# sizhe-li/neural-jacobian-field

Hardware: AMD Instinct MI355X
Metric: rendered rays/s (64 samples/ray, 256^2 image) (higher is better)
Workload: dtype f32 (v_mfma_f32_32x32x2_f32: exact fp32 products, fp32 accumulate -- the reference's arithmetic)

## Files before the change

### include/njf_hip.h

```cpp
#ifndef NJF_HIP_H
#define NJF_HIP_H

#include <stddef.h>
#include <stdint.h>

#ifdef __cplusplus
extern "C" {
#endif

#define NJF_ABI_VERSION 20
#define NJF_MAX_ACTION_DIM 10
#define NJF_HIDDEN 128
#define NJF_LATENT 512
#define NJF_PE_DIM 63
#define NJF_ZDIM 384

#define NJF_RESNET_CHUNKS 22
#define NJF_RESNET_CHUNKS_F16 12
#define NJF_CHUNK_FLOATS 8192
#define NJF_RESNET_W_FLOATS (NJF_RESNET_CHUNKS * NJF_CHUNK_FLOATS)
#define NJF_RESNET_B_FLOATS (10 * 128 + 32)
#define NJF_COLOR_W_FLOATS NJF_CHUNK_FLOATS
#define NJF_COLOR_B_FLOATS (64 + 32)
#define NJF_TRANSFORMER_CHUNKS 7
#define NJF_TRANSFORMER_W_FLOATS (NJF_TRANSFORMER_CHUNKS * NJF_CHUNK_FLOATS)
#define NJF_TRANSFORMER_B_FLOATS (3 * 256 + 32)
#define NJF_QDIM 64

#define NJF_PRECISION_F32 0
#define NJF_PRECISION_F16X2 1
#define NJF_PRECISION_F16F6 2

#define NJF_PRECISION_F16 3

#define NJF_PRECISION_MIXED(d, j) ((d) | (((j) + 1) << 4))

#define NJF_JACOBIAN_NONE 0
#define NJF_JACOBIAN_MLP 1
#define NJF_JACOBIAN_TRANSFORMER 2

typedef struct NjfResnetFcWeights {
  const float* lin_in_w;
  const float* lin_in_b;
  const float* fc0_w[5];
  const float* fc0_b[5];
  const float* fc1_w[5];
  const float* fc1_b[5];
  const float* lin_z_w[3];
  const float* lin_z_b[3];
  const float* lin_out_w;
  const float* lin_out_b;
  int d_out;
} NjfResnetFcWeights;

typedef struct NjfColorHeadWeights {
  const float* w0; const float* b0;
// ... 395 lines not shown
```

### neural-jacobian-field_amd/csrc/njf_device.h

```cpp
#pragma once
#include <hip/hip_runtime.h>
#include <stdint.h>

__device__ __forceinline__ float relu_bits(float x) { return __int_as_float(max(__float_as_int(x), 0)); }

typedef float f32x16 __attribute__((ext_vector_type(16)));
typedef float f32x4 __attribute__((ext_vector_type(4)));
typedef _Float16 f16x8 __attribute__((ext_vector_type(8)));
typedef _Float16 f16x16 __attribute__((ext_vector_type(16)));
typedef _Float16 f16x32 __attribute__((ext_vector_type(32)));
typedef int i32x8 __attribute__((ext_vector_type(8)));
typedef int i32x4 __attribute__((ext_vector_type(4)));
typedef int i32x2 __attribute__((ext_vector_type(2)));
typedef unsigned u32x6 __attribute__((ext_vector_type(6)));

#define PREC_F32 0
#define PREC_F16X2 1
#define PREC_F16F6 2
#define PREC_F16 3

#define NJF_WAVES 4
#define NJF_THREADS (NJF_WAVES * 64)
#define NJF_CHUNK 8192

#define NJF_STREAM_BUFFERS 2
#define LDS_CTR_FLOATS 0
#define LDS_W0 0
#define LDS_W1 NJF_CHUNK
#define LDS_BIAS (NJF_STREAM_BUFFERS * NJF_CHUNK)
#define LDS_BIAS_FLOATS 2752
#define LDS_BIAS_FLOATS_PROPOSAL 1344
#define LDS_SCRATCH_PER_WAVE 528
#define LDS_FLOATS_RENDER (LDS_BIAS + LDS_BIAS_FLOATS + LDS_CTR_FLOATS)
#define LDS_FLOATS_PROPOSAL (LDS_BIAS + LDS_BIAS_FLOATS_PROPOSAL + NJF_WAVES * LDS_SCRATCH_PER_WAVE + LDS_CTR_FLOATS)
#define LDS_SCRATCH_PROPOSAL (LDS_BIAS + LDS_BIAS_FLOATS_PROPOSAL)

extern __shared__ __attribute__((aligned(16))) float njf_lds[];

__device__ __forceinline__ float mfma_step(float a, float b, f32x16& c) {
  c = __builtin_amdgcn_mfma_f32_32x32x2f32(a, b, c, 0, 0, 0);
  return 0.f;
}

#ifdef NJF_STAMPS
#define NJF_STAMP_SLOTS 1024
#ifdef NJF_STAMPS_PROPOSAL
#define NJF_STAMP_BASE LDS_FLOATS_PROPOSAL
#define NJF_STAMP_LOGS_PROPOSAL true
#else
#define NJF_STAMP_BASE LDS_FLOATS_RENDER
#define NJF_STAMP_LOGS_PROPOSAL false
#endif
__device__ unsigned njf_stamp_out[NJF_STAMP_SLOTS];
#define NJF_STAMP_FIELD int stamp_i;
#define NJF_STAMP_INIT(st) (st).stamp_i = -1
#define NJF_STAMP(st, tag)                                                                                   \
  do {                                                                                                       \
    if ((st).stamp_i >= 0 && (st).stamp_i < NJF_STAMP_SLOTS) {                                               \
      njf_lds[NJF_STAMP_BASE + (st).stamp_i] =                                                               \
          __uint_as_float(((unsigned)(tag) << 24) | ((unsigned)__builtin_readcyclecounter() & 0xffffffu));   \
      (st).stamp_i += 1;                                                                                     \
    }                                                                                                        \
  } while (0)
#define NJF_STAMP_P(st, tag) do { if (NJF_STAMP_LOGS_PROPOSAL) NJF_STAMP(st, tag); } while (0)
// ... 129 lines not shown
}
template <bool RELU>
__device__ __forceinline__ void split_pair_u(float x0, float x1, unsigned& hu, unsigned& lu) {
  if (RELU) {
    x0 = relu_bits(x0);
    x1 = relu_bits(x1);
  }
  const f16x2 hp = {(_Float16)x0, (_Float16)x1};
  hu = __builtin_bit_cast(unsigned, hp);
  asm("v_fma_mixlo_f16 %0, -%1, 1.0, %2 op_sel:[0,0,0] op_sel_hi:[1,0,0]" : "=v"(lu) : "v"(hu), "v"(x0));
  asm("v_fma_mixhi_f16 %0, -%1, 1.0, %2 op_sel:[1,0,0] op_sel_hi:[1,0,0]" : "+v"(lu) : "v"(hu), "v"(x1));
}

typedef short s16x2 __attribute__((ext_vector_type(2)));
template <bool RELU>
__device__ __forceinline__ unsigned pack_pair_f16(float x0, float x1) {
  typedef float f32x2 __attribute__((ext_vector_type(2)));
  const f32x2 xp = {x0, x1};
  const f16x2 hp = __builtin_convertvector(xp, f16x2);
  if constexpr (RELU) {
    const s16x2 z = {0, 0};
    return __builtin_bit_cast(unsigned, __builtin_elementwise_max(__builtin_bit_cast(s16x2, hp), z));
  } else {
    return __builtin_bit_cast(unsigned, hp);
  }
}

#define F6_HI 0
#define F6_P1 16384
#define F6_P2 24576
#define F6_SCALE 28672


template <int PREC, int MBO, int NKB, int KB0, bool RELU, int KBI, class ST>
__device__ __forceinline__ void mma_chunk(ST& st, const float* __restrict__ wl, int lane,
                                          const f32x16 (&in)[KBI], f32x16 (&out)[MBO]) {
  constexpr bool SPREAD = MBO == 4 && (NKB == 2 || (PREC == PREC_F16 && NKB == 4)) && NJF_DMA_ROUNDS == 8;
  if constexpr (!SPREAD) stream_flush(st);
  if constexpr (PREC == PREC_F32) {
    const float* base = wl + lane * 4;
#pragma unroll
    for (int kb = 0; kb < NKB; ++kb) {
#pragma unroll
      for (int q = 0; q < 4; ++q) {
        f32x4 a[MBO];
#pragma unroll
        for (int m = 0; m < MBO; ++m) a[m] = *(const f32x4*)(base + ((kb * 4 + q) * MBO + m) * 256);
        if constexpr (SPREAD) {
          if (kb * 4 + q < 4) {
            dma_issue(st, 2 * (kb * 4 + q));
            dma_issue(st, 2 * (kb * 4 + q) + 1);
          }
        }
#pragma unroll
        for (int e = 0; e < 4; ++e) {
          float b = in[KB0 + kb][q * 4 + e];
          if (RELU) b = relu_bits(b);
#pragma unroll
          for (int m = 0; m < MBO; ++m) out[m] = __builtin_amdgcn_mfma_f32_32x32x2f32(a[m][e], b, out[m], 0, 0, 0);
        }
      }
    }
  } else if constexpr (PREC == PREC_F16F6 && MBO == 4 && NKB == 2) {
    typedef __attribute__((address_space(3))) const char* lds_ptr;
    const lds_ptr wb = (lds_ptr)(const char*)wl;
    lds_ptr p16 = wb + lane * 16;
    lds_ptr p8 = wb + lane * 8;
    asm volatile("" : "+v"(p16), "+v"(p8));
    unsigned bh[4][4], bl[4][4], mx[4];
#pragma unroll
    for (int p = 0; p < 4; ++p) {
// ... 690 lines not shown
    for (int m = 0; m < 4; ++m)
#pragma unroll
      for (int q = 0; q < 2; ++q) {
        u32x4 o;
#pragma unroll
        for (int e = 0; e < 4; ++e) o[e] = pack_pair_f16<DO_RELU>(v[m][8 * q + 2 * e], v[m][8 * q + 2 * e + 1]);
        *(u32x4*)(d16 + 16 * m + 8 * q) = o;
      }
  } else {
#pragma unroll
  for (int m = 0; m < 4; ++m)
#pragma unroll
    for (int q = 0; q < 4; ++q) {
      f32x4 o;
#pragma unroll
      for (int e = 0; e < 4; ++e) o[e] = DO_RELU ? fmaxf(v[m][4 * q + e], 0.f) : v[m][4 * q + e];
      *(f32x4*)(dst + 16 * m + 4 * q) = o;
    }
  }
  if (mask != nullptr) {
    unsigned w[2] = {0u, 0u};
#pragma unroll
    for (int m = 0; m < 4; ++m)
#pragma unroll
      for (int r = 0; r < 16; ++r) {
        const unsigned b = (unsigned)min(max(__float_as_int(v[m][r]), 0), 1);
        w[m >> 1] |= b << (16 * (m & 1) + r);
      }
    typedef unsigned u32x2 __attribute__((ext_vector_type(2)));
    *(u32x2*)mask = u32x2{w[0], w[1]};
  }
}

template <int PREC, bool DUMP = false, int SHARED = 0, class ST>
__device__ __forceinline__ void resnet_tile(ST& st, const float* __restrict__ bias,
                                            const float* __restrict__ gz, const PointGeom& g,
                                            const f32x16 (&pe)[2], int wave, int lane, f32x16 (&out)[1],
                                            ActDump dump = ActDump{nullptr, nullptr, 0}, const TileShareF16* share = nullptr) {
  static_assert(SHARED == 0 || (PREC == PREC_F16 && !DUMP), "the shared tile state exists for the plain-fp16 inference kernels");
  const int hh = lane >> 5;
  constexpr bool FUSED = PREC == PREC_F32 && !DUMP;
  f32x16 h[4], net[4];
#pragma unroll
  for (int m = 0; m < 4; ++m) h[m] = (f32x16)(0.f);
  if (DUMP && dump.pe != nullptr) {
#pragma unroll
    for (int kb = 0; kb < 2; ++kb)
#pragma unroll
      for (int q = 0; q < 4; ++q) {
        f32x4 o;
#pragma unroll
        for (int e = 0; e < 4; ++e) o[e] = pe[kb][4 * q + e];
        *(f32x4*)(dump.pe + 16 * kb + 4 * q) = o;
      }
  }
  {
    const float* wl = stream_step(st, wave, lane);
    if constexpr ((SHARED & 1) != 0) mma_lin_in_f16_packed(st, wl, lane, share->pe, h);
    else if constexpr (FUSED) mma_chunk_gather_f32<0, false, 2>(st, wl, lane, pe, h, gz, g);
    else mma_chunk<PREC, 4, 2, 0, false, 2>(st, wl, lane, pe, h);
  }
  if constexpr (PREC == PREC_F16) {
    static_assert(!DUMP, "the plain-fp16 mode is an inference mode (training forwards dump fp32-class activations)");
    Footprint fp_net;
    if constexpr ((SHARED & 2) != 0) point_footprint(g, fp_net);
    for (int blk = 0; blk < 5; ++blk) {
      if (blk < 3) {
        NJF_STAMP(st, 4);
        if constexpr ((SHARED & 2) != 0) add_hoisted_latent_f16<4>((const _Float16*)map_at<PREC>(gz, blk * 128), g, hh, h, &fp_net);
        else add_hoisted_latent<4, PREC>(map_at<PREC>(gz, blk * 128), g, lane, h);
        NJF_STAMP(st, 5);
      }
// ... 15 lines not shown
      NJF_STAMP(st, 4);
      add_hoisted_latent<4, PREC>(gz + blk * 128, g, lane, h);
      NJF_STAMP(st, 5);
    }
    if (DUMP) dump_vec128<true>(dump_layer(dump, 2 * blk), h, dump.mask ? dump.mask + (size_t)(2 * blk) * (dump.stride / 32) : nullptr, dump.half);
    const float* bl = bias + blk * 256;
    bias_init<4, true, PREC>(bl, hh, net);
    {
      {
        const float* wl = stream_step(st, wave, lane);
        mma_chunk<PREC, 4, 2, 0, true, 4>(st, wl, lane, h, net);
      }
      {
        const float* wl = stream_step(st, wave, lane);
        mma_chunk<PREC, 4, 2, 2, true, 4>(st, wl, lane, h, net);
      }
    }
    if (DUMP) dump_vec128<true>(dump_layer(dump, 2 * blk + 1), net, dump.mask ? dump.mask + (size_t)(2 * blk + 1) * (dump.stride / 32) : nullptr, dump.half);
    bias_init<4, false, PREC>(bl + 128, hh, h);
    {
      {
        const float* wl = stream_step(st, wave, lane);
        mma_chunk<PREC, 4, 2, 0, true, 4>(st, wl, lane, net, h);
      }
      {
        const float* wl = stream_step(st, wave, lane);
        bool plain = true;
        if constexpr (FUSED) {
          if (blk < 2) {
            mma_chunk_gather_f32<2, true, 4>(st, wl, lane, net, h, gz + (blk + 1) * 128, g);
            plain = false;
          }
        }
        if (plain) mma_chunk<PREC, 4, 2, 2, true, 4>(st, wl, lane, net, h);
      }
    }
    if (DUMP && dump.feat != nullptr) dump_vec128<false>(dump.feat + (size_t)blk * dump.stride, h);
  }
  if (DUMP) dump_vec128<true>(dump_layer(dump, 10), h, dump.mask ? dump.mask + (size_t)10 * (dump.stride / 32) : nullptr, dump.half);
  bias_init<1, true, PREC>(bias + 1280, hh, out);
  {
    const float* wl = stream_step(st, wave, lane);
    mma_chunk<PREC, 1, 4, 0, true, 4>(st, wl, lane, h, out);
  }
}

struct ColorDump {
  float* in;
  float* act;
  size_t stride;
};

template <bool DO_RELU>
__device__ __forceinline__ void dump_vec32(float* __restrict__ dst, const f32x16 (&v)[2]) {
#pragma unroll
  for (int m = 0; m < 2; ++m)
#pragma unroll
    for (int q = 0; q < 4; ++q) {
      f32x4 o;
#pragma unroll
      for (int e = 0; e < 4; ++e) o[e] = DO_RELU ? fmaxf(v[m][4 * q + e], 0.f) : v[m][4 * q + e];
      *(f32x4*)(dst + 16 * m + 4 * q) = o;
    }
}

template <int PREC, bool DUMP = false, class ST>
__device__ __forceinline__ void color_tile(ST& st, const float* __restrict__ bias, const f32x16 (&cin)[1],
                                           int wave, int lane, f32x16 (&rgb)[1],
                                           ColorDump dump = ColorDump{nullptr, nullptr, 0}) {
  const int hh = lane >> 5;
  const float* wl = stream_step(st, wave, lane);
  f32x16 a[2], b[2];
  a[0] = (f32x16)(0.f);
  a[1] = (f32x16)(0.f);
  mma_chunk<PREC, 2, 1, 0, false, 1>(st, wl, lane, cin, a);
  bias_init<2, true, PREC>(bias, hh, b);
  mma_chunk<PREC, 2, 2, 0, true, 2>(st, wl + 2048, lane, a, b);
  bias_init<1, true, PREC>(bias + 64, hh, rgb);
  mma_chunk<PREC, 1, 2, 0, true, 2>(st, wl + 6144, lane, b, rgb);
  if (DUMP && dump.in != nullptr) {
#pragma unroll
    for (int q = 0; q < 4; ++q) {
      f32x4 o;
#pragma unroll
      for (int e = 0; e < 4; ++e) o[e] = cin[0][4 * q + e];
      *(f32x4*)(dump.in + 4 * q) = o;
    }
    dump_vec32<true>(dump.act, a);
    dump_vec32<true>(dump.act + dump.stride, b);
  }
}

__device__ __forceinline__ float erf_branchless(float a) {
  const float t = fabsf(a), s = a * a;
  float r = fmaf(-1.72853470e-5f, t, 3.83197126e-4f);
  const float u = fmaf(-3.88396438e-3f, t, 2.42546219e-2f);
  r = fmaf(r, s, u);
  r = fmaf(r, t, -1.06777877e-1f);
  r = fmaf(r, t, -6.34846687e-1f);
  r = fmaf(r, t, -1.28717512e-1f);
  r = fmaf(r, t, -t);
  const float hi = copysignf(1.0f - __builtin_amdgcn_exp2f(r * 1.4426950408889634f), a);
  float q = -5.96761703e-4f;
  q = fmaf(q, s, 4.99119423e-3f);
  q = fmaf(q, s, -2.67681349e-2f);
  q = fmaf(q, s, 1.12819925e-1f);
  q = fmaf(q, s, -3.76125336e-1f);
  q = fmaf(q, s, 1.28379166e-1f);
  const float lo = fmaf(q, a, a);
  return t > 0.927734375f ? hi : lo;
}

// ... 198 lines not shown
```

### neural-jacobian-field_amd/csrc/njf_kernels.hip

```cpp
#include <hip/hip_runtime.h>
#include <math.h>
#include <stdint.h>

#include <atomic>
#include <type_traits>

#include "../../include/njf_hip.h"
#include "njf_device.h"

enum {
  NJF_OK = 0,
  NJF_E_NULL = -1,
  NJF_E_SHAPE = -2,
  NJF_E_ACTION_DIM = -3,
  NJF_E_SAMPLES = -4,
  NJF_E_DOUT = -5,
  NJF_E_MODE = -6,
  NJF_E_GMAP = -7,
  NJF_E_VALUE = -8,
};

extern "C" int njf_abi_version(void) { return NJF_ABI_VERSION; }
extern "C" int njf_rays_per_workgroup(void) { return NJF_WAVES; }

// ... 188 lines not shown
      const int ip = lane & 31, kh = lane >> 5;
      const int f = 16 * L.mb * ((ip >> 2) & 1) + 16 * m + (ip & 3) + 4 * (ip >> 3);
      const int k = 16 * L.kb * kh + 8 * t + i8;
      const float v = pack_source(L, f, k);
      const _Float16 hi = (_Float16)v;
      const _Float16 lo = (_Float16)(v - (float)hi);
      const size_t o = ((size_t)(t * L.mb + m) * 2) * 512 + lane * 8 + i8;
      dst[o] = hi;
      dst[o + 512] = lo;
    }
  }
  if (L.bdst != nullptr && blockIdx.x == 0) {
    for (int f = threadIdx.x; f < 32 * L.mb; f += blockDim.x) L.bdst[f] = pack_bias_entry(L, f);
  }
}

__global__ void pack_layer_kernel(PackLayer L) { pack_layer_body(L); }

#define NJF_PACK_BATCH 24
struct PackBatch {
  PackLayer l[NJF_PACK_BATCH];
  unsigned char f6[NJF_PACK_BATCH];
  int count;
};

__global__ void pack_batch_kernel(PackBatch B) {
  const int k = blockIdx.y;
  if (B.f6[k]) pack_layer_f16f6_body(B.l[k]);
  else pack_layer_body(B.l[k]);
}

__global__ void fill_kernel(float* p, int n, float v) {
  for (int i = blockIdx.x * blockDim.x + threadIdx.x; i < n; i += gridDim.x * blockDim.x) p[i] = v;
}

__host__ __device__ inline int njf_hoist_layout(int precision) {
  return precision == NJF_PRECISION_F16F6 ? 1 : (precision == NJF_PRECISION_F16 ? 2 : 0);
}
__host__ __device__ inline int njf_hoist_position(int f, int mb_count, int layout) {
  const int hh = f / (16 * mb_count), r = f % (16 * mb_count);
  const int m = r >> 4;
  if (layout == 0) {
    const int q = (r >> 2) & 3, e = r & 3;
    return 32 * m + 8 * q + 4 * hh + e;
  }
  if (layout == 2) {
    const int q = (r >> 3) & 1, e = r & 7;
    return 32 * m + 16 * q + 8 * hh + e;
  }
  const int e = (r >> 2) & 3, i = r & 3;
  return 16 * mb_count * hh + 16 * m + 4 * i + e;
}

extern "C" int njf_hoisted_channel(int feature, int block_channels, int precision) {
  if (block_channels < 32 || (block_channels & 31) || feature < 0 || feature >= block_channels) return NJF_E_SHAPE;
  if (!valid_base_precision(precision)) return NJF_E_MODE;
  return njf_hoist_position(feature, block_channels / 32, njf_hoist_layout(precision));
}

__global__ void pack_linz_kernel(const float* w0, const float* w1, const float* w2, const float* b0, const float* b1,
                                 const float* b2, float* wz, int ld, float* bz, int layout, const float* fold0,
                                 const float* fold1) {
  const int n = 3 * 128 * 512;
  for (int i = blockIdx.x * blockDim.x + threadIdx.x; i < n; i += gridDim.x * blockDim.x) {
    const int c = i % 384, k = i / 384;
    const int l = c >> 7, f = c & 127;
// ... 46 lines not shown
  }
  if (g_pack_scope != nullptr && g_pack_scope->s == s) {
    g_pack_scope->add(L, f6);
    return;
  }
  if (f6) pack_layer_f16f6_kernel<<<64, 256, 0, s>>>(L);
  else pack_layer_kernel<<<(n + 255) / 256, 256, 0, s>>>(L);
}

extern "C" int njf_pack_resnetfc_ld(const NjfResnetFcWeights* src, float* w_out, float* b_out, float* wz_out, int wz_ld,
                                    float* bz_out, int precision, void* stream) {
  if (!src || !w_out || !b_out) return NJF_E_NULL;
  if (!valid_base_precision(precision)) return NJF_E_MODE;
  const int P = precision;
  if (src->d_out < 1 || src->d_out > 32) return NJF_E_DOUT;
  if (!src->lin_in_w || !src->lin_in_b || !src->lin_out_w || !src->lin_out_b) return NJF_E_NULL;
  for (int i = 0; i < 5; ++i)
    if (!src->fc0_w[i] || !src->fc0_b[i] || !src->fc1_w[i] || !src->fc1_b[i]) return NJF_E_NULL;
  if (P == NJF_PRECISION_F16 && !wz_out) return NJF_E_NULL;
  hipStream_t s = (hipStream_t)stream;
  PackScope scope(s);
  launch_pack(src->lin_in_w, src->lin_in_b, 128, NJF_PE_DIM, 4, 2, 1, P, w_out, nullptr, s);
  const int per_layer = P == NJF_PRECISION_F16 ? 1 : 2;
  for (int i = 0; i < 5; ++i) {
    float* base = w_out + (size_t)(1 + 2 * per_layer * i) * NJF_CHUNK_FLOATS;
    launch_pack(src->fc0_w[i], src->fc0_b[i], 128, 128, 4, 4, 0, P, base, b_out + 256 * i, s);
    const int bias_form = P == NJF_PRECISION_F16 ? (i < 2 ? 2 : 1) : 0;
    launch_pack(src->fc1_w[i], src->fc1_b[i], 128, 128, 4, 4, 0, P, base + per_layer * NJF_CHUNK_FLOATS, b_out + 256 * i + 128, s,
                bias_form);
  }
  float* last = w_out + (size_t)(1 + 10 * per_layer) * NJF_CHUNK_FLOATS;
  launch_pack(src->lin_out_w, src->lin_out_b, src->d_out, 128, 1, 4, 0, P, last, b_out + 1280, s);
  fill_kernel<<<16, 256, 0, s>>>(last + 4096, 4096, 0.f);
  if (wz_out) {
    if (!bz_out || wz_ld < 384) return NJF_E_SHAPE;
    for (int i = 0; i < 3; ++i)
      if (!src->lin_z_w[i] || !src->lin_z_b[i]) return NJF_E_NULL;
    pack_linz_kernel<<<256, 256, 0, s>>>(src->lin_z_w[0], src->lin_z_w[1], src->lin_z_w[2], src->lin_z_b[0],
                                         src->lin_z_b[1], src->lin_z_b[2], wz_out, wz_ld, bz_out, njf_hoist_layout(P),
                                         P == NJF_PRECISION_F16 ? src->fc1_b[0] : nullptr,
                                         P == NJF_PRECISION_F16 ? src->fc1_b[1] : nullptr);
  }
  scope.flush();
  return launch_status();
}

extern "C" int njf_pack_resnetfc(const NjfResnetFcWeights* src, float* w_out, float* b_out, float* wz_out, float* bz_out,
                                 int precision, void* stream) {
  return njf_pack_resnetfc_ld(src, w_out, b_out, wz_out, 384, bz_out, precision, stream);
}

extern "C" int njf_pack_linear(const float* w, const float* b, int d_out, int d_in, int kind, float* w_out, float* b_out,
                               int precision, void* stream) {
  if (!w || !w_out) return NJF_E_NULL;
  if (!valid_base_precision(precision)) return NJF_E_MODE;
  if (d_out < 1 || d_in < 1) return NJF_E_SHAPE;
  if (kind == 1 && (d_in != NJF_PE_DIM || !b)) return NJF_E_SHAPE;
  if (kind != 0 && kind != 1) return NJF_E_MODE;
  const int mb = (d_out + 31) / 32, kb = kind == 1 ? 2 : (d_in + 31) / 32;
  launch_pack(w, b, d_out, d_in, mb, kb, kind, precision, w_out, b_out, (hipStream_t)stream);
  return launch_status();
}

extern "C" int njf_pack_color_head(const NjfColorHeadWeights* src, float* w_out, float* b_out, int precision,
                                   void* stream) {
  if (!src || !w_out || !b_out || !src->w0 || !src->b0 || !src->w1 || !src->b1 || !src->w2 || !src->b2) return NJF_E_NULL;
  if (!valid_base_precision(precision)) return NJF_E_MODE;
  hipStream_t s = (hipStream_t)stream;
  PackScope scope(s);
  launch_pack(src->w0, src->b0, 64, 31, 2, 1, 2, precision, w_out, nullptr, s);
  launch_pack(src->w1, src->b1, 64, 64, 2, 2, 0, precision, w_out + 2048, b_out, s);
  launch_pack(src->w2, src->b2, 3, 64, 1, 2, 0, precision, w_out + 6144, b_out + 64, s);
  scope.flush();
  return launch_status();
}


__device__ __forceinline__ void split8(const float (&x)[8], f16x8& hi, f16x8& lo) {
#pragma unroll
  for (int i = 0; i < 8; ++i) {
    const _Float16 h = (_Float16)x[i];
    hi[i] = h;
    lo[i] = (_Float16)(x[i] - (float)h);
  }
}

typedef unsigned u32x4p __attribute__((ext_vector_type(4)));
template <int KS, bool OUT16 = false>
__global__ void __launch_bounds__(256, 2) project_kernel_f16x2(const float* __restrict__ feats, const float* __restrict__ wz,
                                                            const float* __restrict__ bz, int hw, int n, int ld, int K,
                                                            float* __restrict__ out) {
  constexpr int NS = KS / 16;
  __shared__ u32x4p s_a[2][NS][2][4][64];
  __shared__ u32x4p s_b[2][NS][2][4][64];
  const int tid = threadIdx.x, lane = tid & 63, wave = tid >> 6;
  const int j = lane & 31, kh = lane >> 5;
  const int b = blockIdx.z;
  const int p0 = blockIdx.x * 128, n0 = blockIdx.y * 128;
  const int lr = tid & 127, lk = tid >> 7;
  const float* fa = feats + (size_t)b * K * hw + min(p0 + lr, hw - 1);
  const float* fb = wz + min(n0 + lr, n - 1);
  const int blk = lr >> 5, slot = lk * 32 + (lr & 31);
  const int wm = wave & 1, wn = wave >> 1;
  f32x16 acc[2][2];
#pragma unroll
// ... 686 lines not shown

extern "C" int njf_field_depth_points(const float* depth, int batch, int height, int width, const float* k_inv, const float* c2w,
                                      int kind, float near, float far, float max_jump, int views_per_scene, float* points,
                                      int* kept, void* stream) {
  if (!depth || !k_inv || !c2w || !points || !kept) return NJF_E_NULL;
  if (batch < 1 || height < 1 || width < 1 || (long long)batch * height * width >= (1LL << 31)) return NJF_E_SHAPE;
  if (views_per_scene < 1 || batch % views_per_scene) return NJF_E_SHAPE;
  if (kind != NJF_FIELD_DEPTH_RAY && kind != NJF_FIELD_DEPTH_Z) return NJF_E_VALUE;
  if (!(near >= 0.0f) || !(near < INFINITY) || !(far > near)) return NJF_E_VALUE;
  if (!(max_jump >= 0.0f) || !(max_jump < INFINITY)) return NJF_E_VALUE;
  DepthArgs a;
  a.depth = depth;
  a.k_inv = k_inv;
  a.c2w = c2w;
  a.batch = batch;
  a.height = height;
  a.width = width;
  a.views = views_per_scene;
  a.rays = (long long)height * width;
  a.total = a.rays * batch;
  a.kind = kind;
  a.near = near;
  a.far = far;
  a.max_jump = max_jump;
  a.points = points;
  a.kept = kept;
  hipStream_t s = (hipStream_t)stream;
  hipError_t e = hipMemsetAsync(kept, 0, (size_t)(batch / views_per_scene) * sizeof(int), s);
  if (e != hipSuccess) return (int)e;
  depth_points_kernel<<<(unsigned)((a.total + 255) / 256), 256, 0, s>>>(a);
  return launch_status();
}

template <int PREC>
constexpr int resnet_chunks() { return PREC == PREC_F16 ? NJF_RESNET_CHUNKS_F16 : NJF_RESNET_CHUNKS; }
template <int PREC>
constexpr int resnet_gap_at() { return PREC == PREC_F16 ? NJF_RESNET_CHUNKS_F16 : 0x7fffffff; }
template <int PREC>
constexpr int resnet_gap() { return PREC == PREC_F16 ? NJF_RESNET_CHUNKS - NJF_RESNET_CHUNKS_F16 : 0; }

struct RayCommon {
  const float* origins;
  const float* directions;
  int rays_per_batch;
  int total_rays;
  NjfCameras cams;
  NjfFeatureMap gmap;
};

__device__ __forceinline__ void load_bias_block(const float* __restrict__ src, int n, int dst_off) {
  for (int i = threadIdx.x; i < n; i += NJF_THREADS) njf_lds[LDS_BIAS + dst_off + i] = src[i];
}

__device__ __forceinline__ float alpha_of(float ds) {
  const float series = ds * fmaf(-0.5f * ds, fmaf(-(1.0f / 3.0f) * ds, fmaf(-0.25f * ds, fmaf(-0.2f, ds, 1.0f), 1.0f), 1.0f), 1.0f);
  return ds < 0.0625f ? series : 1.0f - expf(-ds);
}

__device__ __forceinline__ float tile_weights(float delta, float sigma, bool valid, int j, float& carry) {
  const float ds = (valid && delta > 0.f) ? delta * sigma : 0.f;
  const float incl = half_scan(ds, j);
  float excl = __shfl_up(incl, 1, 32);
  if (j == 0) excl = 0.f;
  excl += carry;
  carry += __shfl(incl, 31, 32);
  return alpha_of(ds) * expf(-excl);
}

// ... 72 lines not shown
__device__ __forceinline__ ActDump point_dump(const NjfActivationDump& d, size_t pidx, size_t points, int hh,
                                              const PointGeom& g, int tex0, int texel_stride) {
  float* act = nullptr;
  if (d.act) act = d.act_f16 ? (float*)((_Float16*)d.act + pidx * 128 + 64 * hh) : d.act + pidx * 128 + 64 * hh;
  ActDump dump{act, d.pe + pidx * 64 + 32 * hh, points * 128, d.mask ? d.mask + pidx * 4 + 2 * hh : nullptr, d.act_f16 != 0};
  if (hh == 0 && d.foot_idx != nullptr) {
    Footprint f;
    point_footprint(g, f);
    int* fi = d.foot_idx + pidx * 4;
    fi[0] = tex0 + f.t00 / texel_stride;
    fi[1] = tex0 + f.t01 / texel_stride;
    fi[2] = tex0 + f.t10 / texel_stride;
    fi[3] = tex0 + f.t11 / texel_stride;
    float* fw = d.foot_w + pidx * 4;
    fw[0] = f.w00;
    fw[1] = f.w01;
    fw[2] = f.w10;
    fw[3] = f.w11;
  }
  return dump;
}

template <int PREC, bool DUMP = false>
__global__ void __launch_bounds__(NJF_THREADS, 2) proposal_kernel(ProposalArgs a) {
  const int tid = threadIdx.x;
  const int wave = __builtin_amdgcn_readfirstlane(tid >> 6);
  const int lane = tid & 63, j = lane & 31, hh = lane >> 5;
  const int wg = xcd_remap(blockIdx.x, gridDim.x);
  const int ray = wg * NJF_WAVES + wave;
  const bool ray_ok = ray < a.rc.total_rays;
  const int rayc = min(ray, a.rc.total_rays - 1);
  const int b = rayc / a.rc.rays_per_batch;

  load_bias_block(a.b_pack, NJF_RESNET_B_FLOATS, 0);
  const int tiles = (a.s_in + 31) >> 5;
  WeightStream st;
  stream_begin(st, a.w_pack, resnet_chunks<PREC>(), tiles, wave, lane);
  NJF_STAMP_ARM(st, true, wave);

  CamCtx cam;
  load_ctx(a.rc.cams.ctxt_w2c, a.rc.cams.ctxt_k, b, cam);
  const float near = a.rc.cams.z_near[b], far = a.rc.cams.z_far[b];
  const float ox = a.rc.origins[3 * (size_t)rayc], oy = a.rc.origins[3 * (size_t)rayc + 1],
              oz = a.rc.origins[3 * (size_t)rayc + 2];
  const float dx = a.rc.directions[3 * (size_t)rayc], dy = a.rc.directions[3 * (size_t)rayc + 1],
              dz = a.rc.directions[3 * (size_t)rayc + 2];
  const float* gz = map_at<PREC>(a.rc.gmap.data, (size_t)b * a.rc.gmap.height * a.rc.gmap.width * a.rc.gmap.stride + a.gmap_offset);
  const float* bins = a.bins_in + (a.bins_per_ray ? (size_t)rayc * (a.s_in + 1) : 0);
  float* sc = njf_lds + LDS_SCRATCH_PROPOSAL + wave * LDS_SCRATCH_PER_WAVE;
  const float* bias = njf_lds + LDS_BIAS;

  float carry = 0.f;
  for (int t = 0; t < tiles; ++t) {
    const int s = t * 32 + j;
    const bool valid = s < a.s_in;
    const int sc_i = min(s, a.s_in - 1);
    const float b0 = bins[sc_i], b1 = bins[sc_i + 1];
    const float start = b0 * far + (1.0f - b0) * near;
    const float end = b1 * far + (1.0f - b1) * near;
    const float se = start + end;
    const float px = ox + (dx * se) / 2.0f, py = oy + (dy * se) / 2.0f, pz = oz + (dz * se) / 2.0f;
    PointGeom g;
    point_geometry(cam, px, py, pz, a.rc.gmap.height, a.rc.gmap.width, a.rc.gmap.stride, 0u, g);
    NJF_STAMP_P(st, 10);
    f32x16 pe[2];
    positional_encoding(g.xc, g.yc, g.zc, hh, pe);
    f32x16 out[1];
    ActDump dump{nullptr, nullptr, 0};
    if (DUMP && valid && ray_ok)
      dump = point_dump(a.dump, (size_t)ray * a.s_in + s, (size_t)a.rc.total_rays * a.s_in, hh, g,
                        b * a.rc.gmap.height * a.rc.gmap.width, a.rc.gmap.stride);
    resnet_tile<PREC, DUMP>(st, bias, gz, g, pe, wave, lane, out, dump);
    NJF_STAMP_P(st, 14);
    const float pre = __shfl(out[0][0], j, 64);
    const float sigma = expf(pre - 1.0f);
    const float w = tile_weights(end - start, sigma, valid, j, carry);
    if (valid && hh == 0) {
      float wa = w;
      if (a.anneal != 1.0f) wa = powf(w, a.anneal);
      sc[s] = wa + 0.01f;
      if (ray_ok) {
        if (a.weights_out) a.weights_out[(size_t)ray * a.s_in + s] = w;
        if (a.density_out) a.density_out[(size_t)ray * a.s_in + s] = sigma;
      }
    }
  }
  NJF_STAMP_P(st, 13);
  __syncthreads();
  const float* u = a.u + (a.u_per_ray ? (size_t)rayc * (a.s_out + 1) : 0);
  pdf_resample_ray(sc, bins, a.s_in, u, a.s_out, a.bins_out + (size_t)rayc * (a.s_out + 1), lane, ray_ok);
  NJF_STAMP_FLUSH(st, 15, lane);
}

template <int PREC, int DUMP, int SHARE = 0, class ST>
__device__ __forceinline__ float density_stage(ST& st, const float* __restrict__ gz_d, const PointGeom& g, int wave,
                                               int lane, f32x16 (&geo)[1], ActDump dump, TileShareF16* share = nullptr) {
  const int j = lane & 31, hh = lane >> 5;
  f32x16 pe[2];
  positional_encoding(g.xc, g.yc, g.zc, hh, pe);
  if constexpr (SHARE != 0) {
    share_tile(pe, *share);
    resnet_tile<PREC, false, SHARE>(st, njf_lds + LDS_BIAS, gz_d, g, pe, wave, lane, geo, dump, share);
  } else {
    resnet_tile<PREC, DUMP == 2>(st, njf_lds + LDS_BIAS, gz_d, g, pe, wave, lane, geo, dump);
  }
// ... 88 lines not shown
  float delta, tm, px, py, pz;
};
__device__ __forceinline__ void place_sample(float b0, float b1, float near, float far, float ox,
                                             float oy, float oz, float dx, float dy, float dz, SamplePlace& sp) {
  asm volatile("" : "+v"(b0), "+v"(b1));
  const float start = b0 * far + (1.0f - b0) * near;
  const float end = b1 * far + (1.0f - b1) * near;
  const float se = start + end;
  sp.delta = end - start;
  sp.tm = se / 2.0f;
  sp.px = ox + (dx * se) / 2.0f;
  sp.py = oy + (dy * se) / 2.0f;
  sp.pz = oz + (dz * se) / 2.0f;
}

template <int JKIND, int PREC, int DUMP = 0, bool AF = true, int PRECJ = PREC>
__global__ void __launch_bounds__(NJF_THREADS, 2) render_kernel(RenderArgs a) {
  constexpr bool WITH_J = JKIND != 0;
  constexpr int J_CHUNKS = JKIND == 1 ? resnet_chunks<PRECJ>() : (JKIND == 2 ? NJF_TRANSFORMER_CHUNKS : 0);
  constexpr int J_BIAS = JKIND == 1 ? NJF_RESNET_B_FLOATS : NJF_TRANSFORMER_B_FLOATS;
  const int tid = threadIdx.x;
  const int wave = __builtin_amdgcn_readfirstlane(tid >> 6);
  const int lane = tid & 63, j = lane & 31, hh = lane >> 5;
  const int wg = xcd_remap(blockIdx.x, gridDim.x);
  const int ray = wg * NJF_WAVES + wave;
  const bool ray_ok = ray < a.rc.total_rays;
  const int rayc = min(ray, a.rc.total_rays - 1);
  const int b = rayc / a.rc.rays_per_batch;
  const int S = a.samples;

  load_bias_block(a.b_d, NJF_RESNET_B_FLOATS, 0);
  load_bias_block(a.b_c, NJF_COLOR_B_FLOATS, NJF_RESNET_B_FLOATS);
  if (WITH_J) load_bias_block(a.b_j, J_BIAS, NJF_RESNET_B_FLOATS + NJF_COLOR_B_FLOATS);
  const int tiles = (S + 31) >> 5;
  WeightStreamT<resnet_gap_at<PREC>(), resnet_gap<PREC>()> st;
  stream_begin(st, a.w_all, resnet_chunks<PREC>() + 1 + J_CHUNKS, tiles, wave, lane);
  NJF_STAMP_ARM(st, false, wave);

  CamCtx cam;
  load_ctx(a.rc.cams.ctxt_w2c, a.rc.cams.ctxt_k, b, cam);
  const float near = a.rc.cams.z_near[b], far = a.rc.cams.z_far[b];
  const float ox = a.rc.origins[3 * (size_t)rayc], oy = a.rc.origins[3 * (size_t)rayc + 1],
              oz = a.rc.origins[3 * (size_t)rayc + 2];
  const float dx = a.rc.directions[3 * (size_t)rayc], dy = a.rc.directions[3 * (size_t)rayc + 1],
              dz = a.rc.directions[3 * (size_t)rayc + 2];
  const size_t gbase = (size_t)b * a.rc.gmap.height * a.rc.gmap.width * a.rc.gmap.stride;
  const float* gz_d = map_at<PREC>(a.rc.gmap.data, gbase + a.goff_d);
  const float* gz_j = map_at<PRECJ>(a.rc.gmap.data, gbase + a.goff_j);
  const float* bins = a.bins + (size_t)rayc * (S + 1);
  const int A = a.rc.cams.action_dim;
  const float* action = a.rc.cams.action ? a.rc.cams.action + (size_t)b * A : nullptr;

  float carry = 0.f;
  float acc_rgb[3] = {0.f, 0.f, 0.f}, acc_w = 0.f, acc_wt = 0.f;
  float acc_p[3] = {0.f, 0.f, 0.f}, acc_pw[3] = {0.f, 0.f, 0.f};
  float tmin = 3.0e38f, tmax = -3.0e38f;
  f32x16 acc_j = (f32x16)(0.f);
  const bool want_af = AF && WITH_J && a.out.action_features != nullptr;

  for (int t = 0; t < tiles; ++t) {
    const int s = t * 32 + j;
    const bool valid = s < S;
    const int sc_i = min(s, S - 1);
    const size_t si = (size_t)ray * S + s;
    const bool store = valid && ray_ok;
    const float bin0 = bins[sc_i], bin1 = bins[sc_i + 1];
// ... 376 lines not shown
  }
};
struct StoredNodes : ConstantDirection {
  static constexpr bool COUNTED = true, EXTRAS = false;
  static constexpr int MODES = 0b11100;
  const float* xyz;
  const int* node;
  const int* count;
  int capacity;
  int nodes, total;
  __device__ __forceinline__ int entries() const { return counted_length(count, capacity); }
  __device__ __forceinline__ void point(int i, int& b, float& px, float& py, float& pz) const {
    b = min(max(node[i], 0), total - 1) / nodes;
    px = xyz[3 * (size_t)i], py = xyz[3 * (size_t)i + 1], pz = xyz[3 * (size_t)i + 2];
  }
};

template <class SRC, int MODE, int PREC, int PRECJ = PREC, bool FEAT = false>
__global__ void __launch_bounds__(NJF_THREADS, 2) points_kernel(DecoderArgs a, SRC src) {
  static_assert((SRC::MODES >> MODE) & 1, "a mode this source does not have");
  const int entries = src.entries();
  const int tid = threadIdx.x;
  const int wave = __builtin_amdgcn_readfirstlane(tid >> 6);
  const int lane = tid & 63, j = lane & 31, hh = lane >> 5;
  const int wg = xcd_remap(blockIdx.x, gridDim.x);
  if (SRC::COUNTED && wg * (NJF_WAVES * 32) >= entries) return;
  const int tile = wg * NJF_WAVES + wave;
  const int p = tile * 32 + j;
  const bool ok = p < entries;
  const int pc = min(p, entries - 1);

  load_bias_block(a.b_d, NJF_RESNET_B_FLOATS, 0);
  if (MODE >= 2) load_bias_block(a.b_c, NJF_COLOR_B_FLOATS, NJF_RESNET_B_FLOATS);
  if (MODE == 3) load_bias_block(a.b_j, NJF_RESNET_B_FLOATS, NJF_RESNET_B_FLOATS + NJF_COLOR_B_FLOATS);
  if (MODE == 4) load_bias_block(a.b_j, NJF_TRANSFORMER_B_FLOATS, NJF_RESNET_B_FLOATS + NJF_COLOR_B_FLOATS);
  WeightStreamT<resnet_gap_at<PREC>(), resnet_gap<PREC>()> st;
  stream_begin(st, a.w_all,
               MODE <= 1 ? resnet_chunks<PREC>()
                         : resnet_chunks<PREC>() + 1 + (MODE == 3 ? resnet_chunks<PRECJ>() : (MODE == 4 ? NJF_TRANSFORMER_CHUNKS : 0)),
               1, wave, lane);
  int b;
  float px, py, pz;
  src.point(pc, b, px, py, pz);
  CamCtx cam;
  load_ctx(a.cams.ctxt_w2c, a.cams.ctxt_k, b, cam);
  PointGeom g;
  const unsigned gbase = (unsigned)b * (unsigned)(a.gmap.height * a.gmap.width) * (unsigned)a.gmap.stride;
  point_geometry(cam, px, py, pz, a.gmap.height, a.gmap.width, a.gmap.stride, gbase, g);
  const float* bias = njf_lds + LDS_BIAS;
  if (MODE == 0) {
    f32x16 pe[2], out[1];
    positional_encoding(g.xc, g.yc, g.zc, hh, pe);
    resnet_tile<PREC>(st, bias, map_at<PREC>(a.gmap.data, a.goff_d), g, pe, wave, lane, out);
    if (ok && hh == 0 && (!SRC::EXTRAS || a.density)) a.density[p] = expf(out[0][0] - 1.0f);
  } else {
    const int A = a.cams.action_dim;
    constexpr int JK = MODE >= 3 ? MODE - 2 : 0;
    const ActDump nodump{nullptr, nullptr, 0};
    f32x16 geo[1];
    const float sigma = density_stage<PREC, 0>(st, map_at<PREC>(a.gmap.data, a.goff_d), g, wave, lane, geo, nodump);
    if (ok && hh == 0) {
      if (a.density) a.density[p] = sigma;
      if (SRC::EXTRAS && a.geo) {
#pragma unroll
        for (int r = 0; r < 15; ++r) a.geo[15 * (size_t)p + r] = geo[0][r];
      }
// ... 5686 lines not shown
```

### neural-jacobian-field_amd/hip.py

```python

from __future__ import annotations

import ctypes as C
import math
import os
from typing import Dict, Optional

import torch

_HERE = os.path.dirname(os.path.abspath(__file__))
LIB_PATH = os.environ.get("NJF_HIP_LIB", os.path.join(_HERE, "libnjf_hip.so"))

MAX_ACTION_DIM = 10
ZDIM = 384
RESNET_W_FLOATS = 22 * 8192
RESNET_B_FLOATS = 10 * 128 + 32
COLOR_W_FLOATS = 8192
COLOR_B_FLOATS = 96
TRANSFORMER_W_FLOATS = 7 * 8192
TRANSFORMER_B_FLOATS = 3 * 256 + 32
QDIM = 64
JACOBIAN_NONE, JACOBIAN_MLP, JACOBIAN_TRANSFORMER = 0, 1, 2
PRECISIONS = {"f32": 0, "f16x2": 1, "f16f6": 2, "f16": 3}
REDUCED_PRECISIONS = ("f16",)
DEFAULT_PRECISION = os.environ.get("NJF_PRECISION", "f16f6")
if DEFAULT_PRECISION not in PRECISIONS or DEFAULT_PRECISION in REDUCED_PRECISIONS:
    raise ValueError(f"NJF_PRECISION={DEFAULT_PRECISION!r}: the package default must be one of "
                     f"{sorted(set(PRECISIONS) - set(REDUCED_PRECISIONS))}")


def proposal_precision_for(precision: str) -> str:
    return "f16x2" if precision == "f16f6" else precision


def precision_code(precision: Optional[str], jacobian_precision: Optional[str] = None) -> int:
    name = DEFAULT_PRECISION if precision is None else precision
    if name not in PRECISIONS:
        raise ValueError(f"njf_hip: unknown precision {name!r}; choose from {sorted(PRECISIONS)}")
    code = PRECISIONS[name]
    if jacobian_precision is not None and jacobian_precision != name:
        if jacobian_precision not in PRECISIONS:
            raise ValueError(f"njf_hip: unknown precision {jacobian_precision!r}; choose from {sorted(PRECISIONS)}")
        if "f32" in (name, jacobian_precision) or "f16" in (name, jacobian_precision):
            raise ValueError("njf_hip: mixed decoder precisions exist for the two split-precision modes only")
        code |= (PRECISIONS[jacobian_precision] + 1) << 4
    return code

_vp = C.c_void_p


class ResnetFcWeights(C.Structure):
# ... 1522 lines not shown
```

Measured before the change: 2.019 million.

## Compute fp32 density and colour output heads on VALU from LDS tables

```diff
diff --git a/include/njf_hip.h b/include/njf_hip.h
--- a/include/njf_hip.h
+++ b/include/njf_hip.h
@@ -20,8 +20,10 @@
 #define NJF_CHUNK_FLOATS 8192
 #define NJF_RESNET_W_FLOATS (NJF_RESNET_CHUNKS * NJF_CHUNK_FLOATS)
 #define NJF_RESNET_B_FLOATS (10 * 128 + 32)
+#define NJF_RESNET_HEAD1_TABLE ((NJF_RESNET_CHUNKS - 1) * NJF_CHUNK_FLOATS + NJF_CHUNK_FLOATS / 2)
 #define NJF_COLOR_W_FLOATS NJF_CHUNK_FLOATS
 #define NJF_COLOR_B_FLOATS (64 + 32)
+#define NJF_COLOR_HEAD3_TABLE 6144
 #define NJF_TRANSFORMER_CHUNKS 7
 #define NJF_TRANSFORMER_W_FLOATS (NJF_TRANSFORMER_CHUNKS * NJF_CHUNK_FLOATS)
 #define NJF_TRANSFORMER_B_FLOATS (3 * 256 + 32)
diff --git a/neural-jacobian-field_amd/csrc/njf_device.h b/neural-jacobian-field_amd/csrc/njf_device.h
--- a/neural-jacobian-field_amd/csrc/njf_device.h
+++ b/neural-jacobian-field_amd/csrc/njf_device.h
@@ -28,8 +28,10 @@
 #define LDS_W0 0
 #define LDS_W1 NJF_CHUNK
 #define LDS_BIAS (NJF_STREAM_BUFFERS * NJF_CHUNK)
-#define LDS_BIAS_FLOATS 2752
-#define LDS_BIAS_FLOATS_PROPOSAL 1344
+#define LDS_BIAS_FLOATS 2944
+#define LDS_HEAD3 2720
+#define LDS_BIAS_FLOATS_PROPOSAL 1472
+#define LDS_HEAD1 1312
 #define LDS_SCRATCH_PER_WAVE 528
 #define LDS_FLOATS_RENDER (LDS_BIAS + LDS_BIAS_FLOATS + LDS_CTR_FLOATS)
 #define LDS_FLOATS_PROPOSAL (LDS_BIAS + LDS_BIAS_FLOATS_PROPOSAL + NJF_WAVES * LDS_SCRATCH_PER_WAVE + LDS_CTR_FLOATS)
@@ -225,11 +227,11 @@
 #define F6_SCALE 28672
 
 
-template <int PREC, int MBO, int NKB, int KB0, bool RELU, int KBI, class ST>
+template <int PREC, int MBO, int NKB, int KB0, bool RELU, int KBI, bool DMA = true, class ST>
 __device__ __forceinline__ void mma_chunk(ST& st, const float* __restrict__ wl, int lane,
                                           const f32x16 (&in)[KBI], f32x16 (&out)[MBO]) {
-  constexpr bool SPREAD = MBO == 4 && (NKB == 2 || (PREC == PREC_F16 && NKB == 4)) && NJF_DMA_ROUNDS == 8;
-  if constexpr (!SPREAD) stream_flush(st);
+  constexpr bool SPREAD = DMA && MBO == 4 && (NKB == 2 || (PREC == PREC_F16 && NKB == 4)) && NJF_DMA_ROUNDS == 8;
+  if constexpr (DMA && !SPREAD) stream_flush(st);
   if constexpr (PREC == PREC_F32) {
     const float* base = wl + lane * 4;
 #pragma unroll
@@ -986,12 +988,48 @@
   }
 }
 
-template <int PREC, bool DUMP = false, int SHARED = 0, class ST>
+template <int ROWS, int MB>
+__device__ __forceinline__ void head_rows_valu(const float* __restrict__ b, const float* __restrict__ tbl, int hh,
+                                               const f32x16 (&h)[MB], float (&pre)[ROWS]) {
+  static_assert(MB % 2 == 0, "two chains over MB / 2 blocks each");
+  float acc[ROWS], hi[ROWS];
+#pragma unroll
+  for (int c = 0; c < ROWS; ++c) {
+    acc[c] = hh == 0 ? b[c] : 0.f;
+    hi[c] = 0.f;
+  }
+  const float* w = tbl + 16 * MB * hh;
+#pragma unroll
+  for (int m = 0; m < MB; ++m)
+#pragma unroll
+    for (int q = 0; q < 4; ++q) {
+      f32x4 v[ROWS];
+#pragma unroll
+      for (int c = 0; c < ROWS; ++c) v[c] = *(const f32x4*)(w + c * 32 * MB + 16 * m + 4 * q);
+#pragma unroll
+      for (int e = 0; e < 4; ++e) {
+        const float x = relu_bits(h[m][4 * q + e]);
+#pragma unroll
+        for (int c = 0; c < ROWS; ++c) {
+          if (m < MB / 2) acc[c] = fmaf(x, v[c][e], acc[c]);
+          else hi[c] = fmaf(x, v[c][e], hi[c]);
+        }
+      }
+    }
+#pragma unroll
+  for (int c = 0; c < ROWS; ++c) {
+    const float half = acc[c] + hi[c];
+    pre[c] = half + __shfl_xor(half, 32, 64);
+  }
+}
+
+template <int PREC, bool DUMP = false, int SHARED = 0, bool ROW1 = false, class ST>
 __device__ __forceinline__ void resnet_tile(ST& st, const float* __restrict__ bias,
                                             const float* __restrict__ gz, const PointGeom& g,
                                             const f32x16 (&pe)[2], int wave, int lane, f32x16 (&out)[1],
                                             ActDump dump = ActDump{nullptr, nullptr, 0}, const TileShareF16* share = nullptr) {
   static_assert(SHARED == 0 || (PREC == PREC_F16 && !DUMP), "the shared tile state exists for the plain-fp16 inference kernels");
+  static_assert(!ROW1 || PREC == PREC_F32, "the 1-row head off the stream exists in exact fp32");
   const int hh = lane >> 5;
   constexpr bool FUSED = PREC == PREC_F32 && !DUMP;
   f32x16 h[4], net[4];
@@ -1073,14 +1111,25 @@
             plain = false;
           }
         }
+        if constexpr (ROW1) {
+          if (plain && st.dma_next != 0) {
+            mma_chunk<PREC, 4, 2, 2, true, 4, false>(st, wl, lane, net, h);
+            plain = false;
+          }
+        }
         if (plain) mma_chunk<PREC, 4, 2, 2, true, 4>(st, wl, lane, net, h);
       }
     }
     if (DUMP && dump.feat != nullptr) dump_vec128<false>(dump.feat + (size_t)blk * dump.stride, h);
   }
   if (DUMP) dump_vec128<true>(dump_layer(dump, 10), h, dump.mask ? dump.mask + (size_t)10 * (dump.stride / 32) : nullptr, dump.half);
-  bias_init<1, true, PREC>(bias + 1280, hh, out);
-  {
+  if constexpr (ROW1) {
+    float pre[1];
+    head_rows_valu<1, 4>(bias + 1280, bias + LDS_HEAD1, hh, h, pre);
+    out[0] = (f32x16)(0.f);
+    out[0][0] = pre[0];
+  } else {
+    bias_init<1, true, PREC>(bias + 1280, hh, out);
     const float* wl = stream_step(st, wave, lane);
     mma_chunk<PREC, 1, 4, 0, true, 4>(st, wl, lane, h, out);
   }
@@ -1117,8 +1166,16 @@
   mma_chunk<PREC, 2, 1, 0, false, 1>(st, wl, lane, cin, a);
   bias_init<2, true, PREC>(bias, hh, b);
   mma_chunk<PREC, 2, 2, 0, true, 2>(st, wl + 2048, lane, a, b);
-  bias_init<1, true, PREC>(bias + 64, hh, rgb);
-  mma_chunk<PREC, 1, 2, 0, true, 2>(st, wl + 6144, lane, b, rgb);
+  if constexpr (PREC == PREC_F32) {
+    float pre[3];
+    head_rows_valu<3, 2>(bias + 64, njf_lds + LDS_BIAS + LDS_HEAD3, hh, b, pre);
+    rgb[0] = (f32x16)(0.f);
+#pragma unroll
+    for (int c = 0; c < 3; ++c) rgb[0][c] = pre[c];
+  } else {
+    bias_init<1, true, PREC>(bias + 64, hh, rgb);
+    mma_chunk<PREC, 1, 2, 0, true, 2>(st, wl + 6144, lane, b, rgb);
+  }
   if (DUMP && dump.in != nullptr) {
 #pragma unroll
     for (int q = 0; q < 4; ++q) {
diff --git a/neural-jacobian-field_amd/csrc/njf_kernels.hip b/neural-jacobian-field_amd/csrc/njf_kernels.hip
--- a/neural-jacobian-field_amd/csrc/njf_kernels.hip
+++ b/neural-jacobian-field_amd/csrc/njf_kernels.hip
@@ -244,6 +244,13 @@
 
 __global__ void fill_kernel(float* p, int n, float v) {
   for (int i = blockIdx.x * blockDim.x + threadIdx.x; i < n; i += gridDim.x * blockDim.x) p[i] = v;
+}
+
+__global__ void pack_head_table_kernel(const float* __restrict__ w, int n, float* __restrict__ dst, int dst_n,
+                                       const float* __restrict__ b, int nb, float* __restrict__ bdst, int bdst_n) {
+  for (int i = blockIdx.x * blockDim.x + threadIdx.x; i < dst_n; i += gridDim.x * blockDim.x) dst[i] = i < n ? w[i] : 0.f;
+  if (bdst != nullptr && blockIdx.x == 0)
+    for (int i = threadIdx.x; i < bdst_n; i += blockDim.x) bdst[i] = i < nb ? b[i] : 0.f;
 }
 
 __host__ __device__ inline int njf_hoist_layout(int precision) {
@@ -356,6 +363,9 @@
   float* last = w_out + (size_t)(1 + 10 * per_layer) * NJF_CHUNK_FLOATS;
   launch_pack(src->lin_out_w, src->lin_out_b, src->d_out, 128, 1, 4, 0, P, last, b_out + 1280, s);
   fill_kernel<<<16, 256, 0, s>>>(last + 4096, 4096, 0.f);
+  if (P == NJF_PRECISION_F32)
+    pack_head_table_kernel<<<1, NJF_HIDDEN, 0, s>>>(src->lin_out_w, NJF_HIDDEN, w_out + NJF_RESNET_HEAD1_TABLE, NJF_HIDDEN, nullptr, 0,
+                                                    nullptr, 0);
   if (wz_out) {
     if (!bz_out || wz_ld < 384) return NJF_E_SHAPE;
     for (int i = 0; i < 3; ++i)
@@ -394,7 +404,9 @@
   PackScope scope(s);
   launch_pack(src->w0, src->b0, 64, 31, 2, 1, 2, precision, w_out, nullptr, s);
   launch_pack(src->w1, src->b1, 64, 64, 2, 2, 0, precision, w_out + 2048, b_out, s);
-  launch_pack(src->w2, src->b2, 3, 64, 1, 2, 0, precision, w_out + 6144, b_out + 64, s);
+  if (precision == NJF_PRECISION_F32)
+    pack_head_table_kernel<<<8, 256, 0, s>>>(src->w2, 3 * 64, w_out + NJF_COLOR_HEAD3_TABLE, 2048, src->b2, 3, b_out + 64, 32);
+  else launch_pack(src->w2, src->b2, 3, 64, 1, 2, 0, precision, w_out + 6144, b_out + 64, s);
   scope.flush();
   return launch_status();
 }
@@ -1147,8 +1159,13 @@
   return launch_status();
 }
 
-template <int PREC>
-constexpr int resnet_chunks() { return PREC == PREC_F16 ? NJF_RESNET_CHUNKS_F16 : NJF_RESNET_CHUNKS; }
+template <int PREC, bool ROW1 = false>
+constexpr int resnet_chunks() {
+  static_assert(!ROW1 || PREC == PREC_F32, "the 1-row head off the stream exists in exact fp32");
+  return PREC == PREC_F16 ? NJF_RESNET_CHUNKS_F16 : NJF_RESNET_CHUNKS - (ROW1 ? 1 : 0);
+}
+static_assert(LDS_HEAD1 == NJF_RESNET_B_FLOATS && LDS_HEAD1 + NJF_HIDDEN <= LDS_BIAS_FLOATS_PROPOSAL, "proposal pass: table behind the biases");
+static_assert(LDS_HEAD3 >= 2 * NJF_RESNET_B_FLOATS + NJF_COLOR_B_FLOATS && LDS_HEAD3 + 3 * 64 <= LDS_BIAS_FLOATS, "colour head: table behind every bias block");
 template <int PREC>
 constexpr int resnet_gap_at() { return PREC == PREC_F16 ? NJF_RESNET_CHUNKS_F16 : 0x7fffffff; }
 template <int PREC>
@@ -1287,10 +1304,12 @@
   const int rayc = min(ray, a.rc.total_rays - 1);
   const int b = rayc / a.rc.rays_per_batch;
 
+  constexpr bool ROW1 = PREC == PREC_F32;
   load_bias_block(a.b_pack, NJF_RESNET_B_FLOATS, 0);
+  if constexpr (ROW1) load_bias_block(a.w_pack + NJF_RESNET_HEAD1_TABLE, NJF_HIDDEN, LDS_HEAD1);
   const int tiles = (a.s_in + 31) >> 5;
   WeightStream st;
-  stream_begin(st, a.w_pack, resnet_chunks<PREC>(), tiles, wave, lane);
+  stream_begin(st, a.w_pack, resnet_chunks<PREC, ROW1>(), tiles, wave, lane);
   NJF_STAMP_ARM(st, true, wave);
 
   CamCtx cam;
@@ -1325,7 +1344,7 @@
     if (DUMP && valid && ray_ok)
       dump = point_dump(a.dump, (size_t)ray * a.s_in + s, (size_t)a.rc.total_rays * a.s_in, hh, g,
                         b * a.rc.gmap.height * a.rc.gmap.width, a.rc.gmap.stride);
-    resnet_tile<PREC, DUMP>(st, bias, gz, g, pe, wave, lane, out, dump);
+    resnet_tile<PREC, DUMP, 0, ROW1>(st, bias, gz, g, pe, wave, lane, out, dump);
     NJF_STAMP_P(st, 14);
     const float pre = __shfl(out[0][0], j, 64);
     const float sigma = expf(pre - 1.0f);
@@ -1480,6 +1499,7 @@
   load_bias_block(a.b_d, NJF_RESNET_B_FLOATS, 0);
   load_bias_block(a.b_c, NJF_COLOR_B_FLOATS, NJF_RESNET_B_FLOATS);
   if (WITH_J) load_bias_block(a.b_j, J_BIAS, NJF_RESNET_B_FLOATS + NJF_COLOR_B_FLOATS);
+  if constexpr (PREC == PREC_F32) load_bias_block(a.w_all + NJF_RESNET_W_FLOATS + NJF_COLOR_HEAD3_TABLE, 3 * 64, LDS_HEAD3);
   const int tiles = (S + 31) >> 5;
   WeightStreamT<resnet_gap_at<PREC>(), resnet_gap<PREC>()> st;
   stream_begin(st, a.w_all, resnet_chunks<PREC>() + 1 + J_CHUNKS, tiles, wave, lane);
@@ -1922,6 +1942,7 @@
 
   load_bias_block(a.b_d, NJF_RESNET_B_FLOATS, 0);
   if (MODE >= 2) load_bias_block(a.b_c, NJF_COLOR_B_FLOATS, NJF_RESNET_B_FLOATS);
+  if constexpr (MODE >= 2 && PREC == PREC_F32) load_bias_block(a.w_all + NJF_RESNET_W_FLOATS + NJF_COLOR_HEAD3_TABLE, 3 * 64, LDS_HEAD3);
   if (MODE == 3) load_bias_block(a.b_j, NJF_RESNET_B_FLOATS, NJF_RESNET_B_FLOATS + NJF_COLOR_B_FLOATS);
   if (MODE == 4) load_bias_block(a.b_j, NJF_TRANSFORMER_B_FLOATS, NJF_RESNET_B_FLOATS + NJF_COLOR_B_FLOATS);
   WeightStreamT<resnet_gap_at<PREC>(), resnet_gap<PREC>()> st;
diff --git a/neural-jacobian-field_amd/hip.py b/neural-jacobian-field_amd/hip.py
--- a/neural-jacobian-field_amd/hip.py
+++ b/neural-jacobian-field_amd/hip.py
@@ -15,8 +15,10 @@
 ZDIM = 384
 RESNET_W_FLOATS = 22 * 8192
 RESNET_B_FLOATS = 10 * 128 + 32
+RESNET_HEAD1_TABLE = 21 * 8192 + 4096
 COLOR_W_FLOATS = 8192
 COLOR_B_FLOATS = 96
+COLOR_HEAD3_TABLE = 6144
 TRANSFORMER_W_FLOATS = 7 * 8192
 TRANSFORMER_B_FLOATS = 3 * 256 + 32
 QDIM = 64
```

New measurement: 2.035 million (median of 6 runs). No clear change (+0.8%).
